# jteutenberg/downpore

Measured on AMD Instinct MI355X. Metric: overlaps/sec (all-vs-all PAF), higher is better.
Workload: dtype u64

## Files before the change

### downpore_amd/csrc/dp_env.h

```cpp
#pragma once
#include <climits>
#include <cstdio>
#include <cstdlib>
#include <cstring>
#include <map>
#include <mutex>
#include <set>
#include <string>

namespace dp_env {
enum Kind { VAR, TUNE, DEBUG };
enum When { CALL, CREATE, PROCESS };
struct Setting {
    Kind kind;
    const char* name;
    When when;
    const char* meaning;
};
inline constexpr Setting kSettings[] = {
    {VAR, "DP_TUNE", CALL, "key=value,...: the keys below"},
    {VAR, "DP_DEBUG", CALL, "a,b,...: the tokens below"},
    {VAR, "DP_SCAN_INDEX", CALL, "0/1: forbid / force the resident k-mer position index (default: from 1 Gbase up)"},
    {VAR, "DP_KINDEX_SHARD", CALL, "0/1/force: index built in shares over the communicator never / also over RCCL / also with one rank"},
    {VAR, "DP_KINDEX_WIDE", CALL, "set: index entries of eight bytes throughout"},
    {VAR, "DP_KINDEX_MAX_K", CALL, "n: no index above k = n (at most 14)"},
    {VAR, "DP_KB_MIN_PBITS", CALL, "n: a floor for the index's position bits, at most 32 (tests reach every entry format on small inputs)"},
    {VAR, "DP_KX_BINS_CAP", CALL, "n: capacity of a bin, at least 16 (tests: bins that overflow)"},
    {VAR, "DP_KX_ONESHOT", CALL, "0: count, wait, fill instead of the index step in one go"},
    {VAR, "DP_KX_DENSE", CALL, "0/1: the dense regime's kernels never / always"},
    {VAR, "DP_INDEX_FILL_ROWS", CALL, "0/1: bit matrices by atomics / seed-set rows in LDS + transpose (default: by size)"},
    {VAR, "DP_CHAIN_PASSES", CALL, "n: proposal passes of the chaining stage, 0..6 (default 3; 0 = the serial walk alone)"},
    {VAR, "DP_CHAIN_TIER", CALL, "2/3: the LDS / the one-lane tier for every pair (tests)"},
    {VAR, "DP_CHAIN_PERFECT", CALL, "0: no perfect-chain shortcut"},
    {VAR, "DP_CHAIN_PACK", CALL, "1: chains always packed for a host consumer"},
    {VAR, "DP_CONS_LAYOUTS", CALL, "words nosmall,eager,huge,nohuge: which LDS layouts of the consensus kernel run when (tests)"},
    {VAR, "DP_TRIM_MIDDLE", CALL, "set and not 0: CLI trim and overlap -trim run the middle stage"},
    {VAR, "DP_TRIM_MID_REC_CAP", CALL, "n: first capacity of dp_trim_search's record buffer, at least 1 (tests: the repeat on overflow)"},
    {VAR, "DP_DEVICE_CONSENSUS", CALL, "0: BuildConsensus on the host; 1: where the host builds it, its seed-space alignment on the device"},
    {VAR, "DP_DEVICE_CHUNK", CALL, "0: chunkWorker on the host"},
    {VAR, "DPH_PRECHAIN", CALL, "0/1: the chunk stage behind the un-waited scan never / always (default: up to three slots)"},
    {VAR, "DP_WINDOW_CACHE", CREATE, "0: per-plan dp_select_seeds calls instead of the window cache"},
    {VAR, "DP_EXEC_SLOTS", CREATE, "n: executor slots of the CLI's overlap job (default 8)"},
    {VAR, "DP_HOST_THREADS", PROCESS, "n: size of the worker pool = the CPU budget everything else is derived from (default: cgroup quota)"},
    {VAR, "DPH_PLAN_LANES", CREATE, "n: planner lanes, 1..8, and no adaptive growth"},
    {VAR, "DPH_TEXT_THREADS", CREATE, "n: formatter threads, 1..16"},
    {VAR, "DP_MAP_THREADS", CREATE, "n: host threads a map job deals its reads to"},
    {VAR, "DP_MAP_INFLIGHT", CREATE, "n: reads each of them keeps in flight, at least 64"},
    {VAR, "DP_MAP_SHARDS", CREATE, "n: reference index of a map job in n shards"},
    {VAR, "DP_MAP_DEVICES", CREATE, "a,b,...: the devices that hold them"},
    {VAR, "DP_DEV_CACHE_MB", PROCESS, "n: device bytes that may stay parked after the context that owned the reads (default 16384)"},
    {VAR, "DP_PIN_CACHE_MB", PROCESS, "n: pinned host bytes that may stay parked (default 2048)"},
    {VAR, "DP_KERNEL_TIMING", PROCESS, "n: timing events around every n-th round of a context (default 8, 0 = never); the initial value dp_set_kernel_timing overrides"},
    {VAR, "DP_SPIN_SYNC", CREATE, "0/1: host threads poll / busy-wait for their context's stream (default: dp_set_stream_wait)"},
    {VAR, "DPH_PROFILE", CREATE, "set: host pipeline counters and set-up marks on stderr"},
    {TUNE, "spec_blocks", CALL, "workgroups of the chaining stage's proposal passes (default 1024)"},
    {TUNE, "scan_wg_per_cu", CALL, "persistent scan workgroups per CU, 1..2 (default 2)"},
    {TUNE, "query_split", CALL, "workgroups per query of the query kernel, up to 16 (default 0 = one, which also clears its own rows)"},
    {TUNE, "upload_threads", PROCESS, "helper threads of the shared pinned upload ring, 0..16 (default 4)"},
    {TUNE, "sync_poll_us", CREATE, "sleep between two polls of a waiting host thread (default 20; 0 = blocking wait)"},
    {TUNE, "kb_b1", CALL, "first-digit bits of the sorted index build, 6..10"},
    {TUNE, "plan_depth", CREATE, "plans computed beyond the highest round asked for, at least 1 (default 6)"},
    {TUNE, "issue_window", CREATE, "rounds issued beyond the slots' own, at least 0 (default 10)"},
    {TUNE, "text_pool_mb", PROCESS, "cap of the process-wide pool of PAF text strings (default 512)"},
    {TUNE, "pin_workers", PROCESS, "1/2: pool workers pinned one per physical core / within NUMA node 0"},
    {TUNE, "map_min_reads_per_thread", CREATE, "reads below which a map job starts no further thread (default 2048)"},
    {TUNE, "map_async_upload", CREATE, "1: a map job's reads travel while the first ones are mapped"},
    {TUNE, "map_ascii_upload", CREATE, "1: the mapper sends its reads as ASCII and the device packs them"},
    {TUNE, "kindex_atomic", CALL, "1: the count -> offsets -> atomic scatter build of the position index"},
    {TUNE, "map_one_lane", CALL, "1: dynamicMatch on one lane"},
    {TUNE, "map_seeds_host", CREATE, "1: AddSingleSeeds walked on the host"},
    {TUNE, "pack_scalar", CREATE, "1: the host's packer without its AVX2 path"},
    {TUNE, "host_values", CREATE, "1: k-mer histogram on the GPU, value table on the host"},
    {TUNE, "host_select", CREATE, "1: the speculative seed selection on host threads"},
    {TUNE, "no_planner_thread", CREATE, "1: plans computed on the calling thread"},
    {TUNE, "no_query_prestage", CALL, "1: dp_find_overlaps uploads the queries itself"},
    {TUNE, "no_shard_queries", CALL, "1: every rank of a scan-shard job does every query window"},
    {TUNE, "touch_isa", PROCESS, "0/1/2: the touch test in scalar / AVX2 / AVX-512 code (only what the CPU has), chosen at its first use"},
    {TUNE, "cons_flag_every", CALL, "n: every n-th window of the device consensus goes to the host path"},
    {TUNE, "plan_delay_us", CREATE, "sleep after every plan: flags arrive after the plan has read them"},
    {TUNE, "fail_begin_rank", CALL, "r: rank r's round fails before it reaches any exchange"},
    {TUNE, "comm_fail_rank", CALL, "r: rank r fails before it meets its peers"},
    {TUNE, "query_debug", CALL, "debug bits handed to the query kernel"},
    {TUNE, "scan_debug", CALL, "debug bits handed to the scan kernels"},
    {DEBUG, "alloc", CALL, "one line per growth of a buffer (read where a buffer grows, not per round)"},
    {DEBUG, "kx_bins", CREATE, "how full the index step's bins are (waits for the stream)"},
    {DEBUG, "kx_oneshot", CREATE, "every one-go index step that had to be repeated"},
    {DEBUG, "cons", CREATE, "per-window records of the consensus kernel"},
    {DEBUG, "cons_why", CREATE, "why a window was left to the host path"},
    {DEBUG, "chain_prof", CREATE, "the chaining stage's per-wave phase timers (make PROF=1)"},
    {DEBUG, "chain_paths", CALL, "the chaining stage records which kernel and which path made every pair final (tests: dp_debug_chain_paths)"},
    {DEBUG, "map_prof", CREATE, "the map kernel's phase timers (make PROF=1)"},
    {DEBUG, "planner", CREATE, "plans as they are computed and fetched"},
    {DEBUG, "start", CREATE, "a job's first twelve rounds, in ms since the end of its set-up"},
    {DEBUG, "slow", CREATE, "every round that took its slot more than 3 ms, with where the time went"},
    {DEBUG, "exchange", CREATE, "the slots' turns at a scan-shard job's exchanges"},
    {DEBUG, "segv", PROCESS, "a crashing host thread prints its frames (handlers installed when the library is loaded)"},
    {DEBUG, "sample_prof", PROCESS, "wall-clock sampling of the pipeline's threads (installed when the library is loaded)"},
};

inline bool known(Kind kind, const char* name) {
    for (const Setting& s : kSettings)
        if (s.kind == kind && strcmp(s.name, name) == 0) return true;
    return false;
}
inline void require(Kind kind, const char* name) {
    if (known(kind, name)) return;
    fprintf(stderr, "dp_env: \"%s\" is not in the table of settings (dp_env.h)\n", name);
    abort();
}

struct Tokens {
    Tokens(const char* v, Kind k) : var(v), kind(k) {}
    const char* const var;
    const Kind kind;
    std::mutex mu;
    std::string text;
    bool parsed = false;
    std::map<std::string, std::string> m;
    std::set<std::string> warned;
    const std::map<std::string, std::string>& get() {
        const char* e = getenv(var);
        if (!e) e = "";
        if (parsed && text == e) return m;
        text = e;
        parsed = true;
        m.clear();
        std::string unknown;
        for (size_t at = 0; at <= text.size();) {
            size_t end = text.find(',', at);
            if (end == std::string::npos) end = text.size();
            const std::string tok = text.substr(at, end - at);
            const size_t eq = tok.find('=');
            const std::string key = tok.substr(0, eq);
            at = end + 1;
            if (tok.empty()) continue;
            m[key] = eq == std::string::npos ? "1" : tok.substr(eq + 1);
            if (!known(kind, key.c_str())) unknown += (unknown.empty() ? "" : ", ") + key;
        }
// ... 55 lines not shown
```

### downpore_amd/csrc/dp_overlap.hip

```cpp
#include <algorithm>
#include <cstring>

#include "dp_common.h"

typedef uint64_t u64;


#define C_CURSOR_BYTES 640
__global__ __launch_bounds__(256) void index_fill_kernel(const dp_seq_ref* __restrict__ refs, uint32_t n_seqs,
                                                         const int32_t* __restrict__ segs, u64* __restrict__ posting,
                                                         u64* __restrict__ seedsets, uint32_t W, uint32_t SW,
                                                         const uint32_t* __restrict__ n_seqs_dev) {
    if (n_seqs_dev) n_seqs = *n_seqs_dev;
    const uint32_t waves = gridDim.x * (blockDim.x >> 6);
    const uint32_t gw = blockIdx.x * (blockDim.x >> 6) + (threadIdx.x >> 6);
    const int lane = dp_lane();
    for (uint32_t idx = gw; idx < n_seqs; idx += waves) {
        const dp_seq_ref r = refs[idx];
        for (uint32_t i = lane; i < r.n_seeds; i += 64) {
            uint32_t seed = (uint32_t)segs[r.seg_off + 2 * (uint64_t)i + 1];
            atomicOr(&posting[(uint64_t)seed * W + (idx >> 6)], 1ull << (idx & 63));
            atomicOr(&seedsets[(uint64_t)idx * SW + (seed >> 6)], 1ull << (seed & 63));
        }
    }
// ... 2515 lines not shown
            int c = RFL(sp.c);
            const int spmm = RFL(sp.mm);
            int len;
            bool chained = false;
            uint32_t tier = 0;
            bool haveMask = false;
            u64 aMask = 0;
            if (c < 0) {
                if (aStaged && nSeeds <= 64) {
                    c = chain_prefilter_seeds(L, A.seedsets + (uint64_t)t * A.SW, (int)nSeeds, &aMask);
                    haveMask = true;
                } else {
                    c = chain_prefilter(A.seedsets + (uint64_t)t * A.SW, qs, A.SW);
                }
            }
            pf.pairs++;
            CHAIN_TICK(wprof, pf, tprev, pre)
            if (c < mm) {
                len = 0;
            } else if (spmm == mm) {
                len = RFL(sp.len);
            } else {
                if (DP_PROFILING && A.prof && mode == 2 && lane == 0) {
                    atomicAdd(&A.cursor[20], 1u);
                    if (spmm == -2) atomicAdd(&A.cursor[21], 1u);
                }
                len = chain_pair(L, nodes, A, aSeg, aN, aStaged, qs, qset, t, mm, ca, cb, haveMask, aMask, nullptr, wprof ? &pf : (ChainProf*)nullptr, &tier);
                if (SLIM && len < 0) {
                    if (lane == 0) {
                        PSpec o = {c, -2, 0, 0};
                        A.pspec[p] = o;
                    }
                    break;
                }
                chained = true;
                pf.chained++;
                CHAIN_TICK(wprof, pf, tprev, pair)
            }
            if (A.paths && lane == 0)
                A.pspec[p].pad = (chained ? CPATH_CHAINED | (SLIM ? CPATH_SLIM : 0u) | tier : c >= mm ? sp.pad : 0u) | (spmm == -2 ? CPATH_MARKED : 0u) |
                                 CPATH_KERNEL(mode == 0 ? 1 : 15);
            algBytes += 16ull * A.SW;
            if (c >= mm) algBytes += 4ull * (u64)(aN + (int)(2 * A.refs[t].n_seeds + 1));
            uint32_t off = 0;
            if (len > 0 && !A.pack) {
                off = (uint32_t)(ib + (u64)i * nSeeds);
                algBytes += 8ull * (u64)len;
            } else if (len > 0) {
                if (lane == 0) off = atomicAdd(&A.cursor[0], (uint32_t)len);
                off = (uint32_t)__shfl((int)off, 0, 64);
                if ((u64)off + (u64)len <= (u64)A.int_cap) {
                    __threadfence_block();
                    for (int x = lane; x < len; x += 64) {
                        A.ma[off + x] = ld_agent(&ca[x]);
                        A.mb[off + x] = ld_agent(&cb[x]);
                    }
                } else {
                    if (lane == 0) A.cursor[3] = 1;
                    len = 0;
                }
                algBytes += 8ull * (u64)len;
            }
            if (lane == 0) {
                MRec rec = {q, t, off, (uint32_t)len};
                A.recs[p] = rec;
            }
            if (len > 0 && len * 2 > mm * 3) mm = (len * 2) / 3;
            if (mode == 0 && chained) {
                i++;
                break;
            }
        }
        if (lane == 0) {
            QState st = {mm, i};
            A.qstate[q] = st;
            if (algBytes) atomicAdd((unsigned long long*)(A.cursor + 32) + (q & 63u), (unsigned long long)algBytes);
            if (mode == 0 && i < cnt) A.cursor[8] = 1u;
        }
        CHAIN_TICK(wprof, pf, tprev, out)
    }
    if (wprof && lane == 0) chain_prof_store(A.prof + 16 * ((size_t)A.prof_walk_slot + gw), pf, tkernel0);
}

__global__ __launch_bounds__(64 * S_WAVES) void chain_spec_kernel(const ChainArgs A, const u64* __restrict__ totals) {
    typedef CSlim LW;
    enum { WAVES = S_WAVES };
    __shared__ LW sh[WAVES];
    LW& L = sh[threadIdx.x >> 6];
    const int lane = dp_lane();
    const uint32_t waves = gridDim.x * WAVES;
    const uint32_t gw = blockIdx.x * WAVES + (threadIdx.x >> 6);
    if (A.cursor[3] != 0 || A.cursor[8 + A.pass] == 0) return;
    const uint32_t total = (uint32_t)min(totals[0], (u64)A.pair_cap);
    const bool sprof = DP_PROFILING && A.prof;
    ChainProf pf = {};
    unsigned long long tprev = 0;
    const unsigned long long tkernel0 = sprof ? wall_clock64() : 0ull;
    for (uint32_t p = gw; p < total; p += waves) {
        if (sprof) tprev = wall_clock64();
        const uint32_t q = A.pq[p];
        const uint32_t t = A.clist[p];
        PSpec sp = A.pspec[p];
        const uint32_t pb_ = A.pbase[q], cnt_ = A.qcnt[q];
        const QState st = A.qstate[q];
        const u64 qo0 = A.qoff[q], qo1 = A.qoff[q + 1];
        const u64 ib = A.ibase[q];
        const dp_seq_ref rT = A.refs[min(t, A.n_refs - 1)];
        do {
        const uint32_t i = p - pb_;
        if (i >= cnt_) continue;
        if (i < st.next) continue;
        const int mm = RFL(st.mm);
        if (RFL(sp.mm) == mm) continue;
        if (RFL(sp.mm) == -2) continue;
        const int aN = RFL((int)(qo1 - qo0));
        const uint32_t nSeeds = (uint32_t)aN / 2;
        if (ib + (u64)cnt_ * nSeeds > A.sint_cap) continue;
        const int32_t* aSeg = A.qsegs + qo0;
        const u64* qset = A.qsets + (uint64_t)q * A.SW;
        const bool aStaged = aN <= (int)LW::ACAP;
        pf.pairs++;
        CHAIN_TICK(sprof, pf, tprev, rec)
        const u64* qs = chain_stage_a(L, aSeg, aN, qset, A.SW, aStaged);
        CHAIN_TICK(sprof, pf, tprev, stagea)
        int c = RFL(sp.c);
        bool haveMask = false;
        u64 aMask = 0;
        if (c < 0) {
            if (aStaged && nSeeds <= 64) {
                c = chain_prefilter_seeds(L, A.seedsets + (uint64_t)t * A.SW, (int)nSeeds, &aMask);
                haveMask = true;
            } else {
                c = chain_prefilter(A.seedsets + (uint64_t)t * A.SW, qs, A.SW);
            }
        }
        CHAIN_TICK(sprof, pf, tprev, pre)
        int len = 0, pmm = mm;
        uint32_t tier = 0;
        if (c >= mm) {
            pf.chained++;
            len = chain_pair(L, (CNode*)nullptr, A, aSeg, aN, aStaged, qs, qset, t, mm, A.sa + ib + (u64)i * nSeeds, A.sb + ib + (u64)i * nSeeds,
                             haveMask, aMask, &rT, sprof ? &pf : (ChainProf*)nullptr, &tier);
            if (len < 0) {
                len = 0;
                pmm = -2;
            }
        }
        CHAIN_TICK(sprof, pf, tprev, pair)
        if (lane == 0) {
            PSpec o = {c, pmm, len, (A.paths && c >= mm && pmm != -2) ? (CPATH_CHAINED | CPATH_SLIM | tier) : 0u};
            A.pspec[p] = o;
        }
        __builtin_amdgcn_wave_barrier();
        } while (0);
    }
    if (sprof && lane == 0) chain_prof_store(A.prof + 16 * ((size_t)A.pass * A.prof_stride + gw), pf, tkernel0);
}

__device__ void chain_resolve_query(const ChainArgs& A, uint32_t q, int lane) {
    const uint32_t cnt = A.qcnt[q];
    if (cnt == 0) return;
    const QState st = A.qstate[q];
    int mm = RFL(st.mm);
    uint32_t next = (uint32_t)RFL((int)st.next);
    if (next >= cnt) return;
    const uint32_t pb = A.pbase[q];
    const int aN = RFL((int)(A.qoff[q + 1] - A.qoff[q]));
    const uint32_t nSeeds = (uint32_t)aN / 2;
    const u64 ib = A.ibase[q];
    if ((u64)pb + cnt > (u64)A.pair_cap || ib + (u64)cnt * nSeeds > A.sint_cap) return;
    u64 algBytes = 0;
    bool stopped = false;
    while (next < cnt && !stopped) {
        const uint32_t i = next + lane;
        const bool valid = i < cnt;
        PSpec sp = {-1, -1, 0, 0};
        uint32_t t = 0;
        if (valid) {
            sp = A.pspec[pb + i];
            t = A.clist[pb + i];
        }
        const int nHere = (int)min(64u, cnt - next);
        int stop = nHere;
        u64 chainedMask = 0, hitMask = 0;
        for (int l = 0; l < nHere; l++) {
            const int c = RL(sp.c, l);
            if (c < 0) {
                stop = l;
                break;
            }
            if (c < mm) continue;
            if (RL(sp.mm, l) != mm) {
                stop = l;
                break;
            }
            chainedMask |= 1ull << l;
            const int len = RL(sp.len, l);
            if (len > 0) {
                hitMask |= 1ull << l;
                if (len * 2 > mm * 3) mm = (len * 2) / 3;
            }
        }
        const bool fin = lane < stop;
        const bool hit = fin && ((hitMask >> lane) & 1ull);
        const int myLen = hit ? sp.len : 0;
        uint32_t myOff = (uint32_t)(ib + (u64)i * nSeeds);
        bool room = true;
        if (A.pack) {
            const int incl = wave_incl_sum(myLen);
            const int totalLen = __shfl(incl, 63, 64);
            uint32_t off0 = 0;
            if (totalLen > 0) {
                if (lane == 0) off0 = atomicAdd(&A.cursor[0], (uint32_t)totalLen);
                off0 = (uint32_t)__shfl((int)off0, 0, 64);
            }
            myOff = off0 + (uint32_t)(incl - myLen);
            room = (u64)off0 + (u64)totalLen <= (u64)A.int_cap;
            if (!room && lane == 0) A.cursor[3] = 1;
        }
        if (fin) {
            int wlen = 0;
            if (hit && !A.pack) {
                wlen = myLen;
            } else if (hit && room) {
                const int32_t* ca = A.sa + ib + (u64)i * nSeeds;
                const int32_t* cb = A.sb + ib + (u64)i * nSeeds;
                for (int x = 0; x < myLen; x++) {
                    A.ma[myOff + x] = ca[x];
                    A.mb[myOff + x] = cb[x];
                }
                wlen = myLen;
            }
            MRec rec = {q, t, hit && room ? myOff : 0u, (uint32_t)wlen};
            A.recs[pb + i] = rec;
            if (A.paths) A.pspec[pb + i].pad = (((chainedMask >> lane) & 1ull) ? sp.pad : 0u) | CPATH_KERNEL(2 + A.pass);
            algBytes += 16ull * A.SW + 8ull * (u64)wlen;
            if ((chainedMask >> lane) & 1ull) algBytes += 4ull * (u64)(aN + (int)(2 * A.refs[t].n_seeds + 1));
        }
        next += (uint32_t)stop;
        stopped = stop < nHere;
    }
    unsigned long long ab = algBytes;
#pragma unroll
    for (int d = 32; d > 0; d >>= 1) ab += __shfl_xor(ab, d, 64);
    if (lane == 0) {
        QState o = {mm, next};
        A.qstate[q] = o;
        if (ab) atomicAdd((unsigned long long*)(A.cursor + 32) + (q & 63u), ab);
        if (next < cnt) {
            A.cursor[9 + A.pass] = 1u;
            if (A.pass < 2) atomicAdd(&A.cursor[24 + 2 * A.pass + (q & 1u)], cnt - next);
        }
    }
}

__global__ __launch_bounds__(256) void chain_resolve_kernel(const ChainArgs A) {
    const int lane = dp_lane();
    const uint32_t waves = gridDim.x * (blockDim.x >> 6);
    if (A.cursor[3] != 0 || A.cursor[8 + A.pass] == 0) return;
    for (uint32_t q = blockIdx.x * (blockDim.x >> 6) + (threadIdx.x >> 6); q < A.nq; q += waves) chain_resolve_query(A, q, lane);
}

static size_t query_block_stage(dp_ctx* ctx, const int32_t* q_segs, const uint64_t* q_off, uint32_t nq, double hf, uint32_t* mc_n_out,
                                uint32_t* max_seeds_out, int32_t* mc_last_out, size_t* up_off_out, size_t* up_segs_out) {
    const uint64_t nseg = nq ? q_off[nq] : 0;
    uint32_t maxSeeds = 0;
    for (uint32_t q = 0; q < nq; q++) maxSeeds = std::max<uint32_t>(maxSeeds, (uint32_t)((q_off[q + 1] - q_off[q]) / 2));
    const uint32_t mc_n = std::max<uint32_t>(maxSeeds + 1, 8);
    std::vector<int32_t> mc(mc_n);
    for (uint32_t n = 0; n < mc_n; n++) {
        volatile double prod = hf * (double)n;
        volatile double sum = prod + 0.5;
        mc[n] = (int32_t)sum;
    }
    const size_t up_segs = nseg * 4, up_off = ((size_t)nq + 1) * 8, up_mc = (size_t)mc_n * 4;
    if (dev_reserve(ctx, ctx->d_qsegs, up_off + up_segs + up_mc + 64)) return 0;
    if (pin_reserve(ctx, ctx->h_qup, up_segs + up_off + up_mc + 64)) return 0;
    uint8_t* up = (uint8_t*)ctx->h_qup.p;
    memcpy(up, q_off, up_off);
    memcpy(up + up_off, q_segs, up_segs);
    memcpy(up + up_off + up_segs, mc.data(), up_mc);
    *mc_n_out = mc_n;
    *max_seeds_out = maxSeeds;
    *mc_last_out = mc[maxSeeds];
    *up_off_out = up_off;
    *up_segs_out = up_segs;
    return up_off + up_segs + up_mc;
}

extern "C" int dp_query_prestage(dp_ctx* ctx, const int32_t* q_segs, const uint64_t* q_off, uint32_t n_queries, double hit_fraction) {
    if (!ctx || (n_queries && (!q_segs || !q_off))) return ctx ? dp_fail(ctx, DP_ERR_ARG, "dp_query_prestage: bad arguments") : DP_ERR_ARG;
    ctx->q_pre_bytes = 0;
    ctx->q_pre_fetched = false;
    if (!n_queries) return DP_OK;
    hipSetDevice(ctx->device);
    uint32_t mc_n = 0, maxSeeds = 0;
    int32_t mcLast = 0;
    size_t up_off = 0, up_segs = 0;
    const size_t bytes = query_block_stage(ctx, q_segs, q_off, n_queries, hit_fraction, &mc_n, &maxSeeds, &mcLast, &up_off, &up_segs);
    if (!bytes) return DP_ERR_HIP;
    ctx->q_pre_bytes = bytes;
    ctx->q_pre_nq = n_queries;
    ctx->q_pre_hf = hit_fraction;
    return DP_OK;
}

static int query_stage_sparse(dp_ctx* ctx, uint32_t nq, const uint8_t* up, size_t up_off, size_t up_segs, size_t up_mc, bool on_device, uint32_t mc_n,
                              uint32_t maxSeeds, uint32_t** d_qmeta_out, uint64_t** d_words_out, int32_t** d_mc_out, uint32_t* mc_n_out,
                              uint32_t** d_qcnt_out) {
    const dp_ctx* ix = dp_index_of(ctx);
    const uint32_t W = ctx->W, M = ctx->n_seqs;
    const uint64_t nInts = up_segs / 4;
    if (dev_reserve(ctx, ctx->d_qmeta, (size_t)nq * 16 + (size_t)nq * 8 + (size_t)nq * 4 + (size_t)mc_n * 4 + 64)) return DP_ERR_HIP;
    if (dev_reserve(ctx, ctx->d_cand, (size_t)nq * W * 8 + 64)) return DP_ERR_HIP;
    if (dev_reserve(ctx, ctx->d_wlist, (size_t)(nInts / 2 + 1) * 4 + 64)) return DP_ERR_HIP;
    if (dev_reserve(ctx, ctx->d_cursor, C_CURSOR_BYTES)) return DP_ERR_HIP;
    uint32_t* d_qmeta = (uint32_t*)ctx->d_qmeta.p;
    u64* d_words = (u64*)((uint8_t*)ctx->d_qmeta.p + (size_t)nq * 16);
    uint32_t* d_qcnt = (uint32_t*)((uint8_t*)ctx->d_qmeta.p + (size_t)nq * 24);
    const int32_t* d_mc = (const int32_t*)((const uint8_t*)ctx->d_qsegs.p + up_off + up_segs);
    {
        const dp_zero_region z[3] = {{ctx->d_cand.p, (size_t)nq * W * 8}, {d_qmeta, (size_t)nq * 28}, {ctx->d_cursor.p, C_CURSOR_BYTES}};
        const dp_fetch_region f = {ctx->d_qsegs.p, up, up_off + up_segs + up_mc};
        if (int rc = dp_zero_fetch_regions(ctx, z, 3, &f, on_device ? 0 : 1)) return rc;
    }
    DP_HIP(dp_mark(ctx, 4));
    const uint32_t n_glob = ctx->global_n_seqs ? ctx->global_n_seqs : M;
    hipLaunchKernelGGL((query_sparse_kernel<false>), dim3(nq), dim3(64 * Q_WAVES), 0, ctx->stream, ctx->qsegs_dev, ctx->qoff_dev, nq,
                       (const u64*)ix->d_sp_post_off.p, (const uint32_t*)ix->d_sp_post_ids.p, (const uint32_t*)ix->d_pmeta.p, n_glob, W,
                       d_mc, mc_n, (u64*)ctx->d_cand.p, d_qmeta, d_words, d_qcnt, ctx->word_base, (uint32_t*)nullptr, 0u);
    if (maxSeeds > Q_MAXSETS) {
        const uint32_t stride = std::min<uint32_t>(maxSeeds, Q_BIG_MAXSETS);
        if (dev_reserve(ctx, ctx->d_qbig, (size_t)nq * ((size_t)stride + 2) * Q_BIG_WORDS_PER_SET * 4 + 64)) return DP_ERR_HIP;
        hipLaunchKernelGGL((query_sparse_kernel<true>), dim3(nq), dim3(64 * Q_WAVES), 0, ctx->stream, ctx->qsegs_dev, ctx->qoff_dev, nq,
                           (const u64*)ix->d_sp_post_off.p, (const uint32_t*)ix->d_sp_post_ids.p, (const uint32_t*)ix->d_pmeta.p, n_glob, W,
                           d_mc, mc_n, (u64*)ctx->d_cand.p, d_qmeta, d_words, d_qcnt, ctx->word_base, (uint32_t*)ctx->d_qbig.p, stride);
    }
    if (nq) hipLaunchKernelGGL(window_list_kernel, dim3(std::min<uint32_t>(nq, 16384)), dim3(256), 0, ctx->stream, ctx->qsegs_dev,
                               ctx->qoff_dev, nq, (uint32_t*)ctx->d_wlist.p);
    DP_HIP(hipGetLastError());
    DP_HIP(dp_mark(ctx, 5));
    *d_qmeta_out = d_qmeta;
    *d_words_out = d_words;
// ... 131 lines not shown
    uint32_t* d_pbase = (uint32_t*)(d_ibase + nq + 1);
    QState* d_qstate = (QState*)(d_pbase + nq + 1 + ((nq + 1) & 1));
    {
        const void* before = ctx->d_mrec.p;
        if (dev_reserve(ctx, ctx->d_mrec, (size_t)st.want_pairs * sizeof(MRec))) return DP_ERR_HIP;
        if (ctx->d_mrec.p != before) DP_HIP(hipMemsetAsync(ctx->d_mrec.p, 0, ctx->d_mrec.cap, ctx->stream));
    }
    if (dev_reserve(ctx, ctx->d_pspec, (size_t)st.want_pairs * sizeof(PSpec))) return DP_ERR_HIP;
    if (dev_reserve(ctx, ctx->d_clist, (size_t)st.want_pairs * 8)) return DP_ERR_HIP;
    if (dev_reserve(ctx, ctx->d_sa, (size_t)st.want_sints * 4)) return DP_ERR_HIP;
    if (dev_reserve(ctx, ctx->d_sb, (size_t)st.want_sints * 4)) return DP_ERR_HIP;
    if (dev_reserve(ctx, ctx->d_ma, (size_t)st.want_ints * 4)) return DP_ERR_HIP;
    if (dev_reserve(ctx, ctx->d_mb, (size_t)st.want_ints * 4)) return DP_ERR_HIP;
    st.pair_cap = (uint32_t)std::min<uint64_t>(0xfffffff0ull, st.want_pairs);
    st.sint_cap = st.want_sints;
    st.int_cap = (uint32_t)std::min<uint64_t>(0xfffffff0ull, st.want_ints);
    ChainArgs A;
    A.qsegs = ctx->qsegs_dev;
    A.qoff = ctx->qoff_dev;
    A.nq = nq;
    A.qsets = (const u64*)ctx->d_qsets.p;
    A.qmeta = st.d_qmeta;
    A.qcnt = st.d_qcnt;
    A.cand = (const u64*)ctx->d_cand.p;
    A.refs = (const dp_seq_ref*)ctx->d_seqrefs.p;
    A.segs = (const int32_t*)ctx->d_segs.p;
    A.seedsets = (const u64*)ctx->d_seedsets.p;
    A.W = W;
    A.SW = SW;
    A.mc = st.d_mc;
    A.mc_n = st.mc_n;
    A.k = st.k;
    A.maxLength = (int)st.max_query_len;
    A.tier = st.chain_tier;
    A.pool = (CNode*)ctx->d_pool.p;
    A.pool_stride = chain_pool_stride(st.max_query_len);
    A.pbase = d_pbase;
    A.ibase = d_ibase;
    A.clist = (uint32_t*)ctx->d_clist.p;
    A.pq = A.clist + st.pair_cap;
    A.pass = 0;
    A.pspec = (PSpec*)ctx->d_pspec.p;
    A.qstate = d_qstate;
    A.recs = (MRec*)ctx->d_mrec.p;
    A.sa = (int32_t*)ctx->d_sa.p;
    A.sb = (int32_t*)ctx->d_sb.p;
    A.ma = (int32_t*)ctx->d_ma.p;
    A.mb = (int32_t*)ctx->d_mb.p;
    {
        const bool always_pack = dp_env_tristate("DP_CHAIN_PACK") == 1;
        A.pack = (st.defer_fetch && !always_pack && st.sint_cap < 0xfffffff0ull) ? 0 : 1;
        A.walk_always = dp_env_tristate("DP_CHAIN_PERFECT") == 0 ? 1 : 0;
        A.paths = dp_debug("chain_paths") ? 1 : 0;
        st.paths = A.paths != 0;
        ctx->chains_packed = A.pack != 0;
    }
    A.pair_cap = st.pair_cap;
    A.sint_cap = st.sint_cap;
    A.int_cap = st.int_cap;
    A.cursor = d_cur;
    const uint32_t walk0_blocks = std::max<uint32_t>(1, std::min<uint32_t>(1024, (nq + S_WAVES - 1) / S_WAVES));
    A.n_refs = std::max<uint32_t>(1, ctx->n_seqs);
    A.prof = nullptr;
    A.prof_walk_slot = 0;
    A.prof_stride = 0;
    if (ctx->dbg.chain_prof) {
        const size_t pb = ((size_t)st.passes * st.spec_blocks * S_WAVES + (size_t)walk0_blocks * S_WAVES) * 128;
        if (dev_reserve(ctx, ctx->d_sched, pb + 128)) return DP_ERR_HIP;
        A.prof = (unsigned long long*)ctx->d_sched.p;
        A.prof_walk_slot = (uint32_t)(st.passes * st.spec_blocks * S_WAVES);
        A.prof_stride = st.spec_blocks * S_WAVES;
        DP_HIP(hipMemsetAsync(A.prof, 0, pb, ctx->stream));
    }
    if (st.attempt > 0) DP_HIP(hipMemsetAsync(ctx->d_cursor.p, 0, C_CURSOR_BYTES, ctx->stream));
    DP_HIP(dp_mark(ctx, 6));
    hipLaunchKernelGGL(pair_scan_kernel, dim3(1), dim3(1024), 0, ctx->stream, (const uint32_t*)st.d_qcnt, ctx->qoff_dev, nq, d_pbase,
                       d_ibase, d_totals);
    const uint32_t spec_blocks = st.spec_blocks;
    if (A.tier == 0 && st.passes > 0) {
        hipLaunchKernelGGL((chain_walk_kernel<1>), dim3(walk0_blocks), dim3(64 * S_WAVES), 0, ctx->stream, A, 0);
    } else {
        hipLaunchKernelGGL((chain_walk_kernel<0>), dim3(st.walk_blocks), dim3(64 * C_WAVES), 0, ctx->stream, A, 0);
    }
    for (int ps = 0; ps < st.passes; ps++) {
        A.pass = ps;
        hipLaunchKernelGGL(chain_spec_kernel, dim3(spec_blocks), dim3(64 * S_WAVES), 0, ctx->stream, A, (const u64*)d_totals);
        hipLaunchKernelGGL(chain_resolve_kernel, dim3(std::min<uint32_t>(1024, (nq + 3) / 4)), dim3(256), 0, ctx->stream, A);
    }
    A.pass = st.passes;
    const uint32_t final_blocks = st.passes > 0 ? std::min<uint32_t>(st.walk_blocks, 48) : st.walk_blocks;
    hipLaunchKernelGGL((chain_walk_kernel<0>), dim3(final_blocks), dim3(64 * C_WAVES), 0, ctx->stream, A, 2);
    DP_HIP(hipGetLastError());
    DP_HIP(dp_mark(ctx, 7));
    {
        if (st.defer_fetch && st.attempt == 0) {
            st.fetch_owed = true;
        } else {
            const dp_fetch_region f[2] = {{ctx->h_cursor.p, ctx->d_cursor.p, C_CURSOR_BYTES}, {ctx->h_qm.p, st.d_qmeta, (size_t)nq * 28}};
            if (int rc = dp_zero_fetch_regions(ctx, nullptr, 0, f, 2)) return rc;
        }
    }
    st.attempt++;
    return DP_OK;
}

static int chain_check(dp_ctx* ctx, FindState& st, bool* grow) {
    memcpy(st.cur, ctx->h_cursor.p, 128);
    st.alg_bytes = 0;
    for (int i = 0; i < 64; i++) st.alg_bytes += ((const uint64_t*)((const uint8_t*)ctx->h_cursor.p + 128))[i];
    st.chain_ms += dp_elapsed(ctx, 6, 7);
    uint64_t tot_pairs, tot_sints;
    memcpy(&tot_pairs, &st.cur[16], 8);
    memcpy(&tot_sints, &st.cur[18], 8);
    if (tot_pairs > 0xfffffff0ull) return dp_fail(ctx, DP_ERR_CAPACITY, "more than 2^32 (query, candidate) pairs in one round");
    *grow = false;
    if (tot_pairs > st.pair_cap) {
        st.want_pairs = tot_pairs + tot_pairs / 2 + 1024;
        *grow = true;
    }
    if (tot_sints > st.sint_cap) {
        st.want_sints = tot_sints + tot_sints / 2 + 1024;
        *grow = true;
    }
    if ((uint64_t)st.cur[0] > st.int_cap) {
        st.want_ints = std::max<uint64_t>(st.want_ints * 2, (uint64_t)st.cur[0] + 1024);
        *grow = true;
    }
    if (!*grow && st.cur[3]) return dp_fail(ctx, DP_ERR_STATE, "dp_find_overlaps: overflow flag without a total that exceeds a buffer");
    return DP_OK;
}

static int chain_finish(dp_ctx* ctx, FindState& st) {
    st.pending = false;
    if (ctx->dbg.chain_prof && ctx->d_sched.p) {
        const size_t waves = (size_t)st.spec_blocks * S_WAVES;
        const size_t wwaves = (size_t)std::max<uint32_t>(1, std::min<uint32_t>(1024, (st.nq + S_WAVES - 1) / S_WAVES)) * S_WAVES;
        std::vector<unsigned long long> h(((size_t)st.passes * waves + wwaves) * 16);
        if (hipMemcpy(h.data(), ctx->d_sched.p, h.size() * 8, hipMemcpyDeviceToHost) == hipSuccess) {
            for (int ps = -1; ps < st.passes; ps++) {
                unsigned long long sum[16] = {0}, mx[16] = {0}, t0 = ~0ull, t1 = 0, busiest = 0, mostPairs = 0;
                size_t active = 0;
                for (size_t w = 0; w < (ps < 0 ? wwaves : waves); w++) {
                    const unsigned long long* r = &h[16 * (ps < 0 ? (size_t)st.passes * waves + w : (size_t)ps * waves + w)];
                    if (!r[10]) continue;
                    t0 = std::min(t0, r[10]);
                    t1 = std::max(t1, r[11]);
                    if (!r[0]) continue;
                    active++;
                    for (int i = 0; i < 10; i++) sum[i] += r[i];
                    for (int i = 2; i < 10; i++) mx[i] = std::max(mx[i], r[i]);
                    for (int i = 12; i < 16; i++) sum[i] += r[i];
                    busiest = std::max(busiest, r[11] - r[10]);
                    mostPairs = std::max(mostPairs, r[0]);
                }
                if (!sum[0]) continue;
                const double n = (double)sum[0], nc = (double)std::max<unsigned long long>(1, sum[1]);
                fprintf(stderr, "[chain prof] pass %d (-1 = walk 0; its 'records' include the candidate list): %llu pairs (%llu chained) on %zu waves (at most %llu per wave), kernel span %.1f us, busiest wave %.1f us | us per pair: "
                                "records %.2f stage a %.2f prefilter %.2f chain_pair %.2f | per chained pair: stage b + flags %.2f initial %.2f events + walk %.2f (b events %.2f us; %.1f events; %.1f %% perfect chains) out %.2f\n",
                        ps, sum[0], sum[1], active, mostPairs, (t1 - t0) / 100.0, busiest / 100.0, sum[2] / 100.0 / n, sum[3] / 100.0 / n, sum[4] / 100.0 / n,
                        sum[5] / 100.0 / n, sum[6] / 100.0 / nc, sum[7] / 100.0 / nc, sum[8] / 100.0 / nc, sum[12] / 100.0 / nc, sum[13] / nc, 100.0 * sum[14] / nc, sum[9] / 100.0 / nc);
                {
                    unsigned long long w5[5] = {0, 0, 0, 0, 0};
                    for (size_t w = 0; w < (ps < 0 ? wwaves : waves); w++) {
                        const unsigned long long v = h[16 * (ps < 0 ? (size_t)st.passes * waves + w : (size_t)ps * waves + w) + 15];
                        for (int i = 0; i < 5; i++) w5[i] += (v >> (12 * i)) & 0xfff;
                    }
                    fprintf(stderr, "[chain prof]   walked, not perfect: %llu size limits, %llu event 0 starts no / several chains, %llu start beyond maxBIndex, %llu seed or gap, %llu second start\n",
                            w5[0], w5[1], w5[2], w5[3], w5[4]);
                }
                fprintf(stderr, "[chain prof]   largest per-wave sums, us: records %.1f stage a %.1f prefilter %.1f chain_pair %.1f (stage b %.1f initial %.1f walk %.1f) out %.1f\n",
// ... 44 lines not shown
        if (int rc = chain_enqueue(ctx, *st)) return rc;
        DP_HIP(dp_stream_sync(ctx));
    }
    return chain_finish(ctx, *st);
}
extern "C" int dp_debug_chain_paths(dp_ctx* ctx, uint32_t* out3, uint32_t cap, uint32_t* n_pairs, uint32_t* info4) {
    if (!ctx || !n_pairs || !info4 || (cap && !out3)) return ctx ? dp_fail(ctx, DP_ERR_ARG, "dp_debug_chain_paths: bad arguments") : DP_ERR_ARG;
    const FindState* st = ctx->find_state;
    if (!st || st->pending) return dp_fail(ctx, DP_ERR_STATE, "dp_debug_chain_paths: no finished dp_find_overlaps on this context");
    if (!st->paths) return dp_fail(ctx, DP_ERR_STATE, "dp_debug_chain_paths: the stage ran without DP_DEBUG=chain_paths");
    hipSetDevice(ctx->device);
    uint64_t tp = 0;
    memcpy(&tp, &st->cur[16], 8);
    info4[0] = (uint32_t)st->attempt;
    info4[1] = (uint32_t)st->passes;
    info4[2] = st->cur[2];
    info4[3] = st->pair_cap;
    *n_pairs = (uint32_t)tp;
    if (tp > st->pair_cap) return dp_fail(ctx, DP_ERR_STATE, "dp_debug_chain_paths: the last attempt did not fit its buffers");
    if (tp > cap) return DP_OK;
    DP_HIP(dp_stream_sync(ctx));
    std::vector<uint32_t> pq(tp), cl(tp);
    std::vector<PSpec> sp(tp);
    if (tp) {
        DP_HIP(hipMemcpy(cl.data(), ctx->d_clist.p, tp * 4, hipMemcpyDeviceToHost));
        DP_HIP(hipMemcpy(pq.data(), (const uint32_t*)ctx->d_clist.p + st->pair_cap, tp * 4, hipMemcpyDeviceToHost));
        DP_HIP(hipMemcpy(sp.data(), ctx->d_pspec.p, tp * sizeof(PSpec), hipMemcpyDeviceToHost));
    }
    for (uint64_t p = 0; p < tp; p++) {
        out3[3 * p] = pq[p];
        out3[3 * p + 1] = cl[p];
        out3[3 * p + 2] = sp[p].pad;
    }
    return DP_OK;
}

void dp_find_stats(const dp_ctx* ctx, double* query_ms, double* chain_ms, uint64_t* query_bytes, uint64_t* chain_bytes) {
    const FindState* st = ctx->find_state;
    *query_ms = st ? st->query_ms : 0;
    *chain_ms = st ? (double)st->chain_ms : 0;
    *query_bytes = st ? st->query_bytes : 0;
    *chain_bytes = st ? st->chain_bytes : 0;
}

int dp_find_overlaps_impl(dp_ctx* ctx, const int32_t* q_segs, const uint64_t* q_off, uint32_t nq, double hf, int k,
                          uint32_t max_query_len, int want_candidates, dp_match_batch* out) {
    if (!ctx->round_open) return dp_fail(ctx, DP_ERR_STATE, "dp_find_overlaps before dp_round_begin");
    hipSetDevice(ctx->device);
    memset(out, 0, sizeof(*out));
    out->n_queries = nq;
    ctx->find_valid = false;
    ctx->n_pairs = 0;
    ctx->last_nq = nq;
    ctx->last_k = k;
    if (ctx->find_state) ctx->find_state->pending = false;
    const uint32_t M = ctx->n_seqs;
    if (pin_reserve(ctx, ctx->h_cursor, C_CURSOR_BYTES)) return DP_ERR_HIP;
    if (pin_reserve(ctx, ctx->h_cand_off, ((size_t)nq + 1) * 8)) return DP_ERR_HIP;
    ((uint64_t*)ctx->h_cand_off.p)[0] = 0;
    out->cand_off = (const uint64_t*)ctx->h_cand_off.p;
    if (pin_reserve(ctx, ctx->h_moff, 16)) return DP_ERR_HIP;
    if (pin_reserve(ctx, ctx->h_qm, (size_t)nq * 28 + 16)) return DP_ERR_HIP;
    ((uint64_t*)ctx->h_moff.p)[0] = 0;
    out->off = (const uint64_t*)ctx->h_moff.p;
    if (nq == 0 || M == 0) {
        for (uint32_t q = 0; q <= nq; q++) ((uint64_t*)ctx->h_cand_off.p)[q] = 0;
        return DP_OK;
    }
    if (!ctx->find_state) ctx->find_state = new FindState();
    FindState& st = *ctx->find_state;
    st = FindState();
    st.nq = nq;
    st.k = k;
    st.max_query_len = max_query_len;
    u64* d_words = nullptr;
    int32_t* d_mc = nullptr;
    if (dev_reserve(ctx, ctx->d_cursor, C_CURSOR_BYTES)) return DP_ERR_HIP;
    if (dev_reserve(ctx, ctx->d_pbase, ((size_t)nq + 1) * 4 + ((size_t)nq + 1) * 8 + (size_t)nq * sizeof(QState) + (size_t)nq * 4 + 128)) return DP_ERR_HIP;
    if (int rc = dp_query_stage(ctx, q_segs, q_off, nq, hf, &st.d_qmeta, &d_words, &d_mc, &st.mc_n, &st.d_qcnt)) return rc;
    st.d_mc = d_mc;
    st.chain_tier = (int)dp_env_long("DP_CHAIN_TIER", 0);
    const long pass_env = dp_env_long("DP_CHAIN_PASSES", -1, 0, 6);
    st.passes = pass_env >= 0 ? (int)pass_env : 3;
    if (pass_env < 0 && ctx->chain_open_ahead[1] < 2u) st.passes = 2;
    st.walk_blocks = std::min<uint32_t>(256, (nq + C_WAVES - 1) / C_WAVES);
    st.spec_blocks = 1024;
    st.spec_blocks = (uint32_t)std::max(1L, dp_tune("spec_blocks", st.spec_blocks));
    if (dev_reserve(ctx, ctx->d_pool, (size_t)st.walk_blocks * C_WAVES * chain_pool_stride(st.max_query_len) * sizeof(CNode))) return DP_ERR_HIP;
    st.want_pairs = std::max<uint64_t>(1u << 14, ctx->d_mrec.cap / sizeof(MRec));
    st.want_sints = std::max<uint64_t>(1u << 18, ctx->d_sa.cap / 4);
    st.want_ints = std::max<uint64_t>(1u << 18, ctx->d_ma.cap / 4);
    st.defer_fetch = (want_candidates & 6) == 6;
    if (int rc = chain_enqueue(ctx, st)) return rc;
    if ((want_candidates & 6) == 6) {
        st.pending = true;
        for (uint32_t q = 0; q <= nq; q++) ((uint64_t*)ctx->h_cand_off.p)[q] = 0;
        return DP_OK;
    }
    for (;;) {
        DP_HIP(dp_stream_sync(ctx));
        bool grow = false;
        if (int rc = chain_check(ctx, st, &grow)) return rc;
        if (!grow) break;
        if (int rc = chain_enqueue(ctx, st)) return rc;
    }
    if (int rc = chain_finish(ctx, st)) return rc;
    out->query_kernel_ms = st.query_ms;
    out->chain_kernel_ms = st.chain_ms;
    out->query_bytes = st.query_bytes;
    out->chain_bytes = st.chain_bytes;
    if (want_candidates & 2) {
        for (uint32_t q = 0; q <= nq; q++) ((uint64_t*)ctx->h_cand_off.p)[q] = 0;
        return DP_OK;
    }
    const double qk = out->query_kernel_ms, ck = out->chain_kernel_ms;
    const uint64_t qb = out->query_bytes, cb = out->chain_bytes;
    int rc = dp_fetch_overlaps_impl(ctx, want_candidates & 1, out);
    out->query_kernel_ms = qk;
    out->chain_kernel_ms = ck;
    out->query_bytes = qb;
    out->chain_bytes = cb;
    return rc;
}

int dp_match_anchors_launch(dp_ctx* ctx, const dp_fetch_region* fetch, uint32_t* zero_word) {
    const uint32_t nslots = dp_find_pending(ctx) ? dp_find_pair_cap(ctx) : ctx->n_pairs;
    if (dev_reserve(ctx, ctx->d_manchor, (size_t)nslots * 16 + 32)) return DP_ERR_HIP;
    FindState* fs = ctx->find_state;
    dp_fetch_region owed[2] = {{nullptr, nullptr, 0}, {nullptr, nullptr, 0}};
    if (fs && fs->fetch_owed) {
        owed[0] = {ctx->h_cursor.p, ctx->d_cursor.p, C_CURSOR_BYTES};
        owed[1] = {ctx->h_qm.p, fs->d_qmeta, (size_t)fs->nq * 28};
        fs->fetch_owed = false;
    }
    if (!nslots) {
        if (owed[0].dst)
            if (int rc = dp_zero_fetch_regions(ctx, nullptr, 0, owed, 2)) return rc;
        const dp_zero_region z = {zero_word, 8};
        return (fetch || zero_word) ? dp_zero_fetch_regions(ctx, &z, zero_word ? 1 : 0, fetch, fetch ? 1 : 0) : DP_OK;
    }
    AnchorFetch F;
    const dp_fetch_region* fr[3] = {fetch, owed[0].dst ? &owed[0] : nullptr, owed[1].dst ? &owed[1] : nullptr};
    for (int i = 0; i < 3; i++) {
        F.dst[i] = fr[i] ? (unsigned long long*)fr[i]->dst : nullptr;
        F.src[i] = fr[i] ? (const unsigned long long*)fr[i]->src : nullptr;
        F.n8[i] = fr[i] ? (unsigned long long)((fr[i]->bytes + 7) / 8) : 0ull;
    }
    const u64* d_totals = (const u64*)((const uint8_t*)ctx->d_cursor.p + 64);
    hipLaunchKernelGGL(match_anchor_kernel, dim3(std::min<uint32_t>(8192, (nslots + 3) / 4)), dim3(256), 0, ctx->stream,
                       (const MRec*)ctx->d_mrec.p, (const uint32_t*)d_totals, nslots, (const int32_t*)dp_chain_b(ctx),
                       (const dp_seq_ref*)ctx->d_seqrefs.p, (const int32_t*)ctx->d_segs.p, ctx->last_k, (int32_t*)ctx->d_manchor.p, F,
                       zero_word, (const int32_t*)dp_chain_a(ctx), (const int32_t*)ctx->qsegs_dev, (const u64*)ctx->qoff_dev,
                       (int32_t*)ctx->d_manchor.p + 2 * (size_t)nslots);
    ctx->mcover_off = 2 * (size_t)nslots;
    DP_HIP(hipGetLastError());
    return DP_OK;
}

__global__ __launch_bounds__(256) void chain_pack_kernel(MRec* __restrict__ recs, uint32_t nslots, const int32_t* __restrict__ sa,
                                                         const int32_t* __restrict__ sb, int32_t* __restrict__ ma, int32_t* __restrict__ mb,
                                                         uint32_t* __restrict__ total) {
    const int lane = threadIdx.x & 63;
    const uint32_t waves = gridDim.x * (blockDim.x >> 6);
    for (uint32_t slot = blockIdx.x * (blockDim.x >> 6) + (threadIdx.x >> 6); slot < nslots; slot += waves) {
        const MRec r = recs[slot];
        if (r.len == 0) continue;
        uint32_t off = 0;
// ... 183 lines not shown
```

Measured before the change: 41.29 million.

## Fuse later chaining passes into one per-query persistent tail kernel

```diff
diff --git a/downpore_amd/csrc/dp_env.h b/downpore_amd/csrc/dp_env.h
--- a/downpore_amd/csrc/dp_env.h
+++ b/downpore_amd/csrc/dp_env.h
@@ -54,6 +54,8 @@
     {VAR, "DP_SPIN_SYNC", CREATE, "0/1: host threads poll / busy-wait for their context's stream (default: dp_set_stream_wait)"},
     {VAR, "DPH_PROFILE", CREATE, "set: host pipeline counters and set-up marks on stderr"},
     {TUNE, "spec_blocks", CALL, "workgroups of the chaining stage's proposal passes (default 1024)"},
+    {TUNE, "chain_tail", CALL, "0: one proposal and one resolve launch per later pass instead of chain_tail_kernel (kept for one release)"},
+    {TUNE, "tail_blocks", CALL, "grid cap of chain_tail_kernel, at least 1 (default 1024; tests: more queries than workgroups)"},
     {TUNE, "scan_wg_per_cu", CALL, "persistent scan workgroups per CU, 1..2 (default 2)"},
     {TUNE, "query_split", CALL, "workgroups per query of the query kernel, up to 16 (default 0 = one, which also clears its own rows)"},
     {TUNE, "upload_threads", PROCESS, "helper threads of the shared pinned upload ring, 0..16 (default 4)"},
diff --git a/downpore_amd/csrc/dp_overlap.hip b/downpore_amd/csrc/dp_overlap.hip
--- a/downpore_amd/csrc/dp_overlap.hip
+++ b/downpore_amd/csrc/dp_overlap.hip
@@ -2621,6 +2621,56 @@
     if (wprof && lane == 0) chain_prof_store(A.prof + 16 * ((size_t)A.prof_walk_slot + gw), pf, tkernel0);
 }
 
+template <bool STAGE>
+__device__ __forceinline__ void chain_propose(CSlim& L, const ChainArgs& A, uint32_t q, uint32_t p, uint32_t i, uint32_t t, const PSpec sp,
+                                              const QState st, uint32_t cnt_, u64 qo0, u64 qo1, u64 ib, const dp_seq_ref& rT, bool sprof,
+                                              ChainProf& pf, unsigned long long& tprev) {
+    typedef CSlim LW;
+    const int lane = dp_lane();
+    const int mm = RFL(st.mm);
+    if (RFL(sp.mm) == mm) return;
+    if (RFL(sp.mm) == -2) return;
+    const int aN = RFL((int)(qo1 - qo0));
+    const uint32_t nSeeds = (uint32_t)aN / 2;
+    if (ib + (u64)cnt_ * nSeeds > A.sint_cap) return;
+    const int32_t* aSeg = A.qsegs + qo0;
+    const u64* qset = A.qsets + (uint64_t)q * A.SW;
+    const bool aStaged = aN <= (int)LW::ACAP;
+    pf.pairs++;
+    CHAIN_TICK(sprof, pf, tprev, rec)
+    const u64* qs = STAGE ? chain_stage_a(L, aSeg, aN, qset, A.SW, aStaged) : qset;
+    CHAIN_TICK(sprof, pf, tprev, stagea)
+    int c = RFL(sp.c);
+    bool haveMask = false;
+    u64 aMask = 0;
+    if (c < 0) {
+        if (aStaged && nSeeds <= 64) {
+            c = chain_prefilter_seeds(L, A.seedsets + (uint64_t)t * A.SW, (int)nSeeds, &aMask);
+            haveMask = true;
+        } else {
+            c = chain_prefilter(A.seedsets + (uint64_t)t * A.SW, qs, A.SW);
+        }
+    }
+    CHAIN_TICK(sprof, pf, tprev, pre)
+    int len = 0, pmm = mm;
+    uint32_t tier = 0;
+    if (c >= mm) {
+        pf.chained++;
+        len = chain_pair(L, (CNode*)nullptr, A, aSeg, aN, aStaged, qs, qset, t, mm, A.sa + ib + (u64)i * nSeeds, A.sb + ib + (u64)i * nSeeds,
+                         haveMask, aMask, &rT, sprof ? &pf : (ChainProf*)nullptr, &tier);
+        if (len < 0) {
+            len = 0;
+            pmm = -2;
+        }
+    }
+    CHAIN_TICK(sprof, pf, tprev, pair)
+    if (lane == 0) {
+        PSpec o = {c, pmm, len, (A.paths && c >= mm && pmm != -2) ? (CPATH_CHAINED | CPATH_SLIM | tier) : 0u};
+        A.pspec[p] = o;
+    }
+    __builtin_amdgcn_wave_barrier();
+}
+
 __global__ __launch_bounds__(64 * S_WAVES) void chain_spec_kernel(const ChainArgs A, const u64* __restrict__ totals) {
     typedef CSlim LW;
     enum { WAVES = S_WAVES };
@@ -2645,53 +2695,10 @@
         const u64 qo0 = A.qoff[q], qo1 = A.qoff[q + 1];
         const u64 ib = A.ibase[q];
         const dp_seq_ref rT = A.refs[min(t, A.n_refs - 1)];
-        do {
         const uint32_t i = p - pb_;
         if (i >= cnt_) continue;
         if (i < st.next) continue;
-        const int mm = RFL(st.mm);
-        if (RFL(sp.mm) == mm) continue;
-        if (RFL(sp.mm) == -2) continue;
-        const int aN = RFL((int)(qo1 - qo0));
-        const uint32_t nSeeds = (uint32_t)aN / 2;
-        if (ib + (u64)cnt_ * nSeeds > A.sint_cap) continue;
-        const int32_t* aSeg = A.qsegs + qo0;
-        const u64* qset = A.qsets + (uint64_t)q * A.SW;
-        const bool aStaged = aN <= (int)LW::ACAP;
-        pf.pairs++;
-        CHAIN_TICK(sprof, pf, tprev, rec)
-        const u64* qs = chain_stage_a(L, aSeg, aN, qset, A.SW, aStaged);
-        CHAIN_TICK(sprof, pf, tprev, stagea)
-        int c = RFL(sp.c);
-        bool haveMask = false;
-        u64 aMask = 0;
-        if (c < 0) {
-            if (aStaged && nSeeds <= 64) {
-                c = chain_prefilter_seeds(L, A.seedsets + (uint64_t)t * A.SW, (int)nSeeds, &aMask);
-                haveMask = true;
-            } else {
-                c = chain_prefilter(A.seedsets + (uint64_t)t * A.SW, qs, A.SW);
-            }
-        }
-        CHAIN_TICK(sprof, pf, tprev, pre)
-        int len = 0, pmm = mm;
-        uint32_t tier = 0;
-        if (c >= mm) {
-            pf.chained++;
-            len = chain_pair(L, (CNode*)nullptr, A, aSeg, aN, aStaged, qs, qset, t, mm, A.sa + ib + (u64)i * nSeeds, A.sb + ib + (u64)i * nSeeds,
-                             haveMask, aMask, &rT, sprof ? &pf : (ChainProf*)nullptr, &tier);
-            if (len < 0) {
-                len = 0;
-                pmm = -2;
-            }
-        }
-        CHAIN_TICK(sprof, pf, tprev, pair)
-        if (lane == 0) {
-            PSpec o = {c, pmm, len, (A.paths && c >= mm && pmm != -2) ? (CPATH_CHAINED | CPATH_SLIM | tier) : 0u};
-            A.pspec[p] = o;
-        }
-        __builtin_amdgcn_wave_barrier();
-        } while (0);
+        chain_propose<true>(L, A, q, p, i, t, sp, st, cnt_, qo0, qo1, ib, rT, sprof, pf, tprev);
     }
     if (sprof && lane == 0) chain_prof_store(A.prof + 16 * ((size_t)A.pass * A.prof_stride + gw), pf, tkernel0);
 }
@@ -2798,6 +2805,60 @@
     const uint32_t waves = gridDim.x * (blockDim.x >> 6);
     if (A.cursor[3] != 0 || A.cursor[8 + A.pass] == 0) return;
     for (uint32_t q = blockIdx.x * (blockDim.x >> 6) + (threadIdx.x >> 6); q < A.nq; q += waves) chain_resolve_query(A, q, lane);
+}
+
+#define TAIL_BLOCKS 1024
+
+__global__ __launch_bounds__(64 * S_WAVES) void chain_tail_kernel(const ChainArgs A0, const int passes) {
+    typedef CSlim LW;
+    enum { WAVES = S_WAVES };
+    __shared__ LW sh[WAVES];
+    __shared__ QState shq;
+    __shared__ uint32_t shgo;
+    const uint32_t w = threadIdx.x >> 6;
+    LW& L = sh[w];
+    const int lane = dp_lane();
+    ChainArgs A = A0;
+    if (threadIdx.x == 0) shgo = (A.cursor[3] != 0 || A.cursor[9] == 0) ? 0u : 1u;
+    __syncthreads();
+    if (shgo == 0) return;
+    ChainProf pf = {};
+    unsigned long long tprev = 0;
+    for (uint32_t q = blockIdx.x; q < A.nq; q += gridDim.x) {
+        const uint32_t cnt = A.qcnt[q];
+        QState st = A.qstate[q];
+        const uint32_t pb = A.pbase[q];
+        const u64 qo0 = A.qoff[q], qo1 = A.qoff[q + 1];
+        const u64 ib = A.ibase[q];
+        if (cnt == 0 || st.next >= cnt) continue;
+        const int aN = RFL((int)(qo1 - qo0));
+        if ((u64)pb + cnt > (u64)A.pair_cap || ib + (u64)cnt * ((uint32_t)aN / 2) > A.sint_cap) continue;
+        chain_stage_a(L, A.qsegs + qo0, aN, A.qsets + (uint64_t)q * A.SW, A.SW, aN <= (int)LW::ACAP);
+        for (int ps = 1; ps < passes; ps++) {
+            for (uint32_t i = st.next + w; i < cnt; i += WAVES) {
+                const uint32_t p = pb + i;
+                const uint32_t t = A.clist[p];
+                const PSpec sp = A.pspec[p];
+                const dp_seq_ref rT = A.refs[min(t, A.n_refs - 1)];
+                chain_propose<false>(L, A, q, p, i, t, sp, st, cnt, qo0, qo1, ib, rT, false, pf, tprev);
+            }
+            __builtin_amdgcn_fence(__ATOMIC_RELEASE, "workgroup");
+            asm volatile("s_waitcnt vmcnt(0)" ::: "memory");
+            __syncthreads();
+            __builtin_amdgcn_fence(__ATOMIC_ACQUIRE, "workgroup");
+            if (w == 0) {
+                A.pass = ps;
+                chain_resolve_query(A, q, lane);
+                if (lane == 0) shq = A.qstate[q];
+            }
+            __builtin_amdgcn_fence(__ATOMIC_RELEASE, "workgroup");
+            asm volatile("s_waitcnt vmcnt(0)" ::: "memory");
+            __syncthreads();
+            __builtin_amdgcn_fence(__ATOMIC_ACQUIRE, "workgroup");
+            st = shq;
+            if (st.next >= cnt) break;
+        }
+    }
 }
 
 static size_t query_block_stage(dp_ctx* ctx, const int32_t* q_segs, const uint64_t* q_off, uint32_t nq, double hf, uint32_t* mc_n_out,
@@ -3095,10 +3156,16 @@
     } else {
         hipLaunchKernelGGL((chain_walk_kernel<0>), dim3(st.walk_blocks), dim3(64 * C_WAVES), 0, ctx->stream, A, 0);
     }
-    for (int ps = 0; ps < st.passes; ps++) {
+    const bool tail = A.tier == 0 && st.passes >= 2 && dp_tune("chain_tail", 1) != 0 && !ctx->dbg.chain_prof;
+    for (int ps = 0; ps < (tail ? 1 : st.passes); ps++) {
         A.pass = ps;
         hipLaunchKernelGGL(chain_spec_kernel, dim3(spec_blocks), dim3(64 * S_WAVES), 0, ctx->stream, A, (const u64*)d_totals);
         hipLaunchKernelGGL(chain_resolve_kernel, dim3(std::min<uint32_t>(1024, (nq + 3) / 4)), dim3(256), 0, ctx->stream, A);
+    }
+    if (tail) {
+        const uint32_t tail_cap = (uint32_t)std::max(1L, std::min<long>(TAIL_BLOCKS, dp_tune("tail_blocks", TAIL_BLOCKS)));
+        A.pass = 1;
+        hipLaunchKernelGGL(chain_tail_kernel, dim3(std::min<uint32_t>(nq, tail_cap)), dim3(64 * S_WAVES), 0, ctx->stream, A, st.passes);
     }
     A.pass = st.passes;
     const uint32_t final_blocks = st.passes > 0 ? std::min<uint32_t>(st.walk_blocks, 48) : st.walk_blocks;
@@ -3309,7 +3376,6 @@
     st.chain_tier = (int)dp_env_long("DP_CHAIN_TIER", 0);
     const long pass_env = dp_env_long("DP_CHAIN_PASSES", -1, 0, 6);
     st.passes = pass_env >= 0 ? (int)pass_env : 3;
-    if (pass_env < 0 && ctx->chain_open_ahead[1] < 2u) st.passes = 2;
     st.walk_blocks = std::min<uint32_t>(256, (nq + C_WAVES - 1) / C_WAVES);
     st.spec_blocks = 1024;
     st.spec_blocks = (uint32_t)std::max(1L, dp_tune("spec_blocks", st.spec_blocks));
```

New measurement: 39.31 million. -4.8%, worse.
